# dscripka/openWakeWord

Measured on NVIDIA H100. Metric: 80ms audio-frames/sec (concurrent streams), higher is better.
Workload: dtype f16 operands / f32 accumulate (mel, BN, LayerNorm, sigmoid in f32; heads' first layer as fp16 hi/lo split = f32-grade)

## Files before the change

### include/owwb200.h

```cpp
#ifndef OWWB200_H
#define OWWB200_H

#include <stddef.h>
#include <stdint.h>

#ifdef __cplusplus
extern "C" {
#endif

#define OWW_OK            0
#define OWW_EINVAL      (-1)
#define OWW_ECUDA       (-2)
#define OWW_ENOMEM      (-3)
#define OWW_EUNSUPPORTED (-4)

#define OWW_SAMPLES_PER_CHUNK 1280
#define OWW_MEL_BINS            32
#define OWW_WINDOW_ROWS         76
#define OWW_EMBEDDING_DIM       96
#define OWW_INIT_FEATURE_ROWS   41
#define OWW_MAX_HEAD_LAYERS      8

#define OWW_CNN_FP32_WINDOW       0
#define OWW_CNN_TC_WINDOW         2
// ... 111 lines not shown
                      int32_t* h_staged, int16_t* d_staged, int64_t staged_stride, int16_t* d_hist, void* stream);
int oww_ingest_import(oww_ctx* ctx, const int32_t* h_stream_ids, int n, const int32_t* h_rates, const int64_t* h_consumed,
                      const int32_t* h_staged, const int16_t* d_staged, int64_t staged_stride, const int16_t* d_hist,
                      void* stream);

int oww_embed_clips(oww_ctx* ctx, const int16_t* d_pcm, int n_clips, int n_samples, float* d_emb, void* stream);
int oww_predict_clips(oww_ctx* ctx, const int16_t* d_pcm, int n_clips, int n_samples, int pad_samples,
                      const float* h_feature_init, int n_rows, float* d_scores, void* stream);
int oww_clip_schedule(int chunk_size, int64_t n_padded_samples, int32_t* h_chunks_per_call, int max);
int oww_predict_clips_ragged(oww_ctx* ctx, const int16_t* d_pcm, const int64_t* h_offsets, int n_clips, int pad_samples,
                             int chunk_size, const float* h_feature_init, int n_rows, float* d_scores, uint8_t* d_stepped,
                             float* d_emb, void* stream);
int oww_predict_clips_streams(oww_ctx* ctx, const int16_t* d_pcm, const int64_t* h_offsets, int n_clips, int pad_samples,
                              int chunk_size, const float* h_feature_init, int n_rows, float* d_scores, uint8_t* d_stepped,
                              float* d_emb, const int32_t* h_clip_streams, void* stream);
int oww_clip_slab_plan(oww_ctx* ctx, const int32_t* h_steps, int n_clips, int64_t* h_steps_computed, int64_t* h_steps_needed);
int oww_resample_clip_plan(int rate, int64_t n_in, int pad_samples, int64_t* n_out);
int oww_resample_clips(oww_ctx* ctx, const int16_t* d_in, const int64_t* h_in_offsets, const int32_t* h_rates, int n_clips,
                       int pad_samples, int16_t* d_out, const int64_t* h_out_offsets, void* stream);

typedef struct oww_mix_params {
    int32_t fg, bg, rir;
    int32_t reserved;
    int64_t fg_start, fg_len;
    int64_t bg_offset;
    int64_t start;
    double snr_db;
    double volume;
} oww_mix_params;
int oww_mix_clips(oww_ctx* ctx, const int16_t* d_fg, const int64_t* h_fg_off, int n_fg,
                  const int16_t* d_bg, const int64_t* h_bg_off, int n_bg,
                  const float* d_rir, const int64_t* h_rir_off, int n_rir,
                  const oww_mix_params* h_params, int n_mix, int64_t n_samples,
                  int16_t* d_out, uint8_t* d_valid, void* stream);

int oww_metrics_false_positives(oww_ctx* ctx, const float* d_scores, int64_t series_stride, int n_series, int n_frames,
                                const double* h_thresholds, int n_thresholds, int grouping_window, int32_t* h_counts, void* stream);
int oww_metrics_false_positives_f64(oww_ctx* ctx, const double* d_scores, int64_t series_stride, int n_series, int n_frames,
                                    const double* h_thresholds, int n_thresholds, int grouping_window, int32_t* h_counts,
                                    void* stream);
int oww_metrics_count_ge(oww_ctx* ctx, const float* d_scores, int64_t n, const double* h_thresholds, int n_thresholds,
                         uint64_t* h_counts, void* stream);
int oww_metrics_count_ge_f64(oww_ctx* ctx, const double* d_scores, int64_t n, const double* h_thresholds, int n_thresholds,
                             uint64_t* h_counts, void* stream);

int oww_debug_layer(oww_ctx* ctx, const float* d_windows, int n, int layer, float* d_out, void* stream);

int oww_debug_inc_plan(oww_ctx* ctx, int group, int n_streams, int32_t* out, int max_ints);
int oww_debug_inc_cut_plan(oww_ctx* ctx, int group, int n_streams, int n_layers, int32_t* out, int max_ints);

int oww_debug_inc_clocks(oww_ctx* ctx, int64_t* h_unused);
int oww_debug_inc_clocks_read(oww_ctx* ctx, int64_t* h_out104);
int oww_debug_heads_clocks(oww_ctx* ctx, int64_t* h_out64);

int oww_peer_alloc(oww_ctx* ctx, size_t bytes, void** d_ptr, unsigned char handle_out[64]);
int oww_peer_free(oww_ctx* ctx, void* d_ptr);
int oww_peer_open(oww_ctx* ctx, const unsigned char handle[64], void** d_ptr);
int oww_peer_close(oww_ctx* ctx, void* d_ptr);
int oww_peer_copy(oww_ctx* ctx, void* d_dst, const void* d_src, size_t bytes, void* stream);
int oww_peer_signal(oww_ctx* ctx, uint64_t* d_flag, uint64_t value, void* stream);
int oww_peer_wait(oww_ctx* ctx, const uint64_t* d_flags, int n, int stride, uint64_t value, double timeout_s, void* stream);
int oww_peer_status(oww_ctx* ctx, int* timed_out);

uint64_t oww_launch_count(const oww_ctx* ctx);
int oww_enable_stage_timing(oww_ctx* ctx, int n_slots);
int oww_stage_ms(oww_ctx* ctx, float out_ms[3]);

#ifdef __cplusplus
}
#endif
#endif
```

### openwakeword_b200/_native.py

```python
import ctypes as C
import os

import numpy as np

_HERE = os.path.dirname(os.path.abspath(__file__))
LIB_PATH = os.path.join(_HERE, "csrc", "libowwb200.so")
MAX_HEAD_LAYERS = 8

CNN_FP32_WINDOW = 0
CNN_FP32_INCREMENTAL = 1
CNN_TC_WINDOW = 2
CNN_TC_INCREMENTAL = 3


class Config(C.Structure):
    _fields_ = [("device", C.c_int32), ("max_chunks", C.c_int32), ("cnn_mode", C.c_int32),
                ("window_batch", C.c_int32), ("reserved", C.c_int32 * 4)]


class HeadDesc(C.Structure):
    _fields_ = [("n_in", C.c_int32), ("n_layers", C.c_int32), ("dims", C.c_int32 * (MAX_HEAD_LAYERS + 1)),
                ("layernorm", C.c_int32), ("final_act", C.c_int32)]


# ... 28 lines not shown
    "oww_fit_verifiers": (C.c_int, [_P, _P, C.c_int64, C.c_int, _P, _P, _P, C.c_int, C.c_double, C.c_int, C.c_double,
                                    _P, _P, _P, _P, _P, _P, _P]),
    "oww_load_verifiers": (C.c_int, [_P, C.c_int, _P, C.c_int, _P, _P, _P, _P]),
    "oww_add_head_bank": (C.c_int, [_P, C.POINTER(HeadDesc), C.c_int, C.POINTER(C.c_int)]),
    "oww_load_bank_head": (C.c_int, [_P, C.c_int, C.c_int, _P, C.c_size_t]),
    "oww_assign_bank_head": (C.c_int, [_P, C.c_int, _P, C.c_int, _P, _P]),
    "oww_set_head_bank_clip_slot": (C.c_int, [_P, C.c_int, C.c_int]),
    "oww_bank_head_predict": (C.c_int, [_P, C.c_int, C.c_int, _P, C.c_int, _P, _P]),
    "oww_n_heads": (C.c_int, [_P]),
    "oww_n_outputs": (C.c_int, [_P]),
    "oww_melspectrogram": (C.c_int, [_P, _P, C.c_int, C.c_int, _P, C.c_int, _P]),
    "oww_embed_windows": (C.c_int, [_P, _P, C.c_int, _P, _P]),
    "oww_head_predict": (C.c_int, [_P, C.c_int, _P, C.c_int, _P, _P]),
    "oww_set_streams": (C.c_int, [_P, C.c_int]),
    "oww_n_streams": (C.c_int, [_P]),
    "oww_reset": (C.c_int, [_P, _P, C.c_int, _P, C.c_int]),
    "oww_reset_async": (C.c_int, [_P, _P, C.c_int, _P, C.c_int, _P]),
    "oww_step": (C.c_int, [_P, _P, C.c_int64, C.c_int, _P, _P]),
    "oww_step_host": (C.c_int, [_P, _P, C.c_int64, C.c_int, _P]),
    "oww_step_host_submit": (C.c_int, [_P, _P, C.c_int64, C.c_int, C.POINTER(C.c_int)]),
    "oww_step_host_collect": (C.c_int, [_P, C.c_int, _P]),
    "oww_step_ragged": (C.c_int, [_P, _P, C.c_int64, _P, _P, _P]),
    "oww_step_host_ragged": (C.c_int, [_P, _P, C.c_int64, _P, _P]),
    "oww_step_host_ragged_submit": (C.c_int, [_P, _P, C.c_int64, _P, C.POINTER(C.c_int)]),
    "oww_get_features": (C.c_int, [_P, C.c_int, C.c_int, C.c_int, _P]),
    "oww_get_mel": (C.c_int, [_P, C.c_int, C.c_int, _P]),
    "oww_get_counts": (C.c_int, [_P, C.c_int, C.POINTER(C.c_int), C.POINTER(C.c_int)]),
    "oww_stream_state_info": (C.c_int, [_P, C.POINTER(C.c_size_t), C.POINTER(C.c_uint64)]),
    "oww_export_streams": (C.c_int, [_P, _P, C.c_int, _P, _P]),
    "oww_import_streams": (C.c_int, [_P, _P, C.c_int, _P, _P]),
    "oww_stream_state_status": (C.c_int, [_P, C.POINTER(C.c_int)]),
    "oww_set_detector": (C.c_int, [_P, C.POINTER(DetectLabel), C.c_int, C.c_double]),
    "oww_detect": (C.c_int, [_P, _P, C.c_int, _P, _P, _P, C.c_int, _P, _P]),
    "oww_detect_clips": (C.c_int, [_P, C.POINTER(DetectLabel), C.c_int, C.c_double, _P, _P, C.c_float, _P, C.c_int, C.c_int,
                                   _P, _P, C.c_int, _P, _P]),
    "oww_detector_export": (C.c_int, [_P, _P, C.c_int, _P, _P, _P]),
    "oww_detector_import": (C.c_int, [_P, _P, C.c_int, _P, _P, _P]),
    "oww_set_audio_history": (C.c_int, [_P, C.c_int]),
    "oww_get_audio": (C.c_int, [_P, _P, _P, C.c_int, C.c_int, _P, _P, _P]),
    "oww_capture_events": (C.c_int, [_P, _P, _P, C.c_int, C.c_int, _P, _P, _P]),
    "oww_audio_export": (C.c_int, [_P, _P, C.c_int, _P, _P, _P]),
    "oww_audio_import": (C.c_int, [_P, _P, C.c_int, _P, _P, _P]),
    "oww_set_input_rates": (C.c_int, [_P, _P, C.c_int, _P, _P]),
    "oww_ingest": (C.c_int, [_P, _P, _P, _P, _P, _P, _P]),
    "oww_ingest_capacity": (C.c_int, [_P, _P]),
    "oww_ingest_plan": (C.c_int, [C.c_int, C.c_int, C.c_int64, C.c_int, C.c_int64, C.POINTER(C.c_int64),
                                  C.POINTER(C.c_int32), C.POINTER(C.c_int32), C.POINTER(C.c_int64)]),
    "oww_resampler_taps": (C.c_int, [C.c_int, _P, C.c_int, C.POINTER(C.c_int), C.POINTER(C.c_int)]),
    "oww_ingest_export": (C.c_int, [_P, _P, C.c_int, _P, _P, _P, _P, C.c_int64, _P, _P]),
    "oww_ingest_import": (C.c_int, [_P, _P, C.c_int, _P, _P, _P, _P, C.c_int64, _P, _P]),
    "oww_embed_clips": (C.c_int, [_P, _P, C.c_int, C.c_int, _P, _P]),
    "oww_predict_clips": (C.c_int, [_P, _P, C.c_int, C.c_int, C.c_int, _P, C.c_int, _P, _P]),
    "oww_clip_schedule": (C.c_int, [C.c_int, C.c_int64, _P, C.c_int]),
    "oww_predict_clips_ragged": (C.c_int, [_P, _P, _P, C.c_int, C.c_int, C.c_int, _P, C.c_int, _P, _P, _P, _P]),
    "oww_predict_clips_streams": (C.c_int, [_P, _P, _P, C.c_int, C.c_int, C.c_int, _P, C.c_int, _P, _P, _P, _P, _P]),
    "oww_clip_slab_plan": (C.c_int, [_P, _P, C.c_int, C.POINTER(C.c_int64), C.POINTER(C.c_int64)]),
    "oww_resample_clip_plan": (C.c_int, [C.c_int, C.c_int64, C.c_int, C.POINTER(C.c_int64)]),
    "oww_resample_clips": (C.c_int, [_P, _P, _P, _P, C.c_int, C.c_int, _P, _P, _P]),
    "oww_mix_clips": (C.c_int, [_P, _P, _P, C.c_int, _P, _P, C.c_int, _P, _P, C.c_int, _P, C.c_int, C.c_int64, _P, _P, _P]),
    "oww_debug_layer": (C.c_int, [_P, _P, C.c_int, C.c_int, _P, _P]),
    "oww_debug_inc_plan": (C.c_int, [_P, C.c_int, C.c_int, _P, C.c_int]),
    "oww_debug_inc_cut_plan": (C.c_int, [_P, C.c_int, C.c_int, C.c_int, _P, C.c_int]),
    "oww_debug_inc_clocks": (C.c_int, [_P, _P]),
    "oww_debug_inc_clocks_read": (C.c_int, [_P, _P]),
    "oww_debug_heads_clocks": (C.c_int, [_P, _P]),
    "oww_peer_alloc": (C.c_int, [_P, C.c_size_t, C.POINTER(C.c_void_p), C.c_char_p]),
    "oww_peer_free": (C.c_int, [_P, _P]),
    "oww_peer_open": (C.c_int, [_P, C.c_char_p, C.POINTER(C.c_void_p)]),
    "oww_peer_close": (C.c_int, [_P, _P]),
    "oww_peer_copy": (C.c_int, [_P, _P, _P, C.c_size_t, _P]),
    "oww_peer_signal": (C.c_int, [_P, _P, C.c_uint64, _P]),
    "oww_peer_wait": (C.c_int, [_P, _P, C.c_int, C.c_int, C.c_uint64, C.c_double, _P]),
    "oww_peer_status": (C.c_int, [_P, C.POINTER(C.c_int)]),
    "oww_metrics_false_positives": (C.c_int, [_P, _P, C.c_int64, C.c_int, C.c_int, _P, C.c_int, C.c_int, _P, _P]),
    "oww_metrics_false_positives_f64": (C.c_int, [_P, _P, C.c_int64, C.c_int, C.c_int, _P, C.c_int, C.c_int, _P, _P]),
    "oww_metrics_count_ge": (C.c_int, [_P, _P, C.c_int64, _P, C.c_int, _P, _P]),
    "oww_metrics_count_ge_f64": (C.c_int, [_P, _P, C.c_int64, _P, C.c_int, _P, _P]),
    "oww_launch_count": (C.c_uint64, [_P]),
    "oww_enable_stage_timing": (C.c_int, [_P, C.c_int]),
    "oww_stage_ms": (C.c_int, [_P, _P]),
}
EXPORTED_SYMBOLS = tuple(_SIGNATURES)

_lib = None


def load_library():
    global _lib
    if _lib is not None:
        return _lib
    if not os.path.exists(LIB_PATH):
        raise ImportError(
            f"{LIB_PATH} is missing: the CUDA extension has not been built. Run "
            "`python -c 'import __graft_entry__ as g; g.build()'` at the repo root (nvcc, sm_90a). "
            "There is no CPU fallback for the b200 backend.")
    lib = C.CDLL(LIB_PATH)
    for name, (res, args) in _SIGNATURES.items():
        fn = getattr(lib, name)
        fn.restype = res
        fn.argtypes = args
    _lib = lib
    return lib


class NativeError(RuntimeError):
    pass


class ArgumentError(NativeError, ValueError):
    """A buffer the library would read or write out of bounds, refused in Python before the call.  A ValueError, and a
    NativeError like the library's own refusal of a short stride, so callers that catch either keep working."""


def clip_schedule(chunk_size, n_padded_samples):
    lib = load_library()
    n = lib.oww_clip_schedule(int(chunk_size), int(n_padded_samples), None, 0)
    if n < 0:
        raise NativeError(f"oww_clip_schedule failed ({n}): {lib.oww_last_error(None).decode()}")
    out = np.zeros(n, np.int32)
    if n:
        lib.oww_clip_schedule(int(chunk_size), int(n_padded_samples), _ptr(out), n)
    return out


def clip_slab_plan(steps, ctx=None):
    lib = load_library()
    st = np.ascontiguousarray(steps, np.int32)
    done, need = C.c_int64(0), C.c_int64(0)
    n = lib.oww_clip_slab_plan(ctx, _ptr(st), st.size, C.byref(done), C.byref(need))
    if n < 0:
        raise NativeError(f"oww_clip_slab_plan failed ({n})")
    return n, done.value, need.value


def resampler_taps(rate):
    lib = load_library()
    up, down = C.c_int(0), C.c_int(0)
    n = lib.oww_resampler_taps(int(rate), None, 0, C.byref(up), C.byref(down))
    if n < 0:
        raise ValueError(f"sample rate {rate} Hz is not supported: the input rates are 8000, 11025, 12000, 16000, 22050, "
                         "24000, 32000, 44100 and 48000 Hz")
    taps = np.zeros(n, np.float32)
    if n:
        lib.oww_resampler_taps(int(rate), _ptr(taps), n, None, None)
    return taps, up.value, down.value


def ingest_plan(rate, max_chunks, n_before, staged, n_in):
    lib = load_library()
    n_out, chunks, after, max_in = C.c_int64(0), C.c_int32(0), C.c_int32(0), C.c_int64(0)
    rc = lib.oww_ingest_plan(int(rate), int(max_chunks), int(n_before), int(staged), int(n_in), C.byref(n_out),
                             C.byref(chunks), C.byref(after), C.byref(max_in))
    if rc and n_in <= max_in.value:
        raise ValueError(f"oww_ingest_plan refused rate {rate}")
    if rc:
        return None, None, None, max_in.value
    return n_out.value, chunks.value, after.value, max_in.value


def resample_clip_plan(rate, n_in, pad_samples):
    lib = load_library()
    n = C.c_int64(0)
    if lib.oww_resample_clip_plan(int(rate), int(n_in), int(pad_samples), C.byref(n)):
        raise ValueError(f"oww_resample_clip_plan refused rate {rate}, {n_in} samples, pad {pad_samples}: the rates are "
                         "8000, 11025, 12000, 16000, 22050, 24000, 32000, 44100 and 48000 Hz, and the padding a multiple "
                         "of 640 samples (40 ms)")
    return n.value


def _ptr(a):
    if a is None:
        return None
    if isinstance(a, int):
        return a
    if isinstance(a, np.ndarray):
        return a.ctypes.data
    return a.data_ptr()
# ... 700 lines not shown
```

### openwakeword_b200/csrc/heads_grp.cu

```cuda
#include "oww_internal.h"
#include "heads_mma.cuh"
#include <algorithm>
#include <cmath>
#include <cstring>

namespace {

constexpr int kHgThreads = 9 * 32;
constexpr int kHgTile = 128;
constexpr int kHgMaxStages = 6;
constexpr int kHgChunkK = 32;
constexpr int kHgAPlane = 4 * kHgTile * 16;
constexpr int kHgABytes = 2 * kHgAPlane;
constexpr int kHgTileBytes = 3 * kHgABytes;
constexpr int kHgSmem = 227 * 1024;
constexpr int kHgRing0 = 1024;

__device__ __forceinline__ void hg_warp_wait(uint32_t bar, uint32_t parity, int lane) {
    if (lane == 0) mbar_wait(bar, parity);
    __syncwarp();
}
__device__ __forceinline__ void hg_split8(const float* x, uint4& hi, uint4& lo) { hm_split8(x, hi, lo); }

__global__ void __launch_bounds__(256) feat16_sync_kernel(const float* __restrict__ ring, int64_t ring_stride, int rows_mask,
                                                          const int* __restrict__ count, const int* __restrict__ ids, int n,
                                                          int depth, int pos, int NS, int n_tiles, uint8_t* __restrict__ out) {
    const int64_t total = (int64_t)n * 12 * depth;
    oww_pdl_sync();
    for (int64_t i = (int64_t)blockIdx.x * 256 + threadIdx.x; i < total; i += (int64_t)gridDim.x * 256) {
        const int lb = (int)(i % n);
        const int j = (int)((i / n) % 12);
        const int k = (int)(i / ((int64_t)n * 12));
        const int b = ids ? ids[lb] : lb;
        const int row = count[b] - 1 - k;
        float x[8];
        if (row >= 0) {
            const float4* p = reinterpret_cast<const float4*>(ring + (int64_t)b * ring_stride + (int64_t)(row & rows_mask) * 96 + j * 8);
            const float4 u = __ldcg(p), v = __ldcg(p + 1);
            x[0] = u.x; x[1] = u.y; x[2] = u.z; x[3] = u.w; x[4] = v.x; x[5] = v.y; x[6] = v.z; x[7] = v.w;
        } else {
#pragma unroll
            for (int e = 0; e < 8; ++e) x[e] = 0.f;
        }
        uint4 hi, lo;
        hg_split8(x, hi, lo);
        int slot = (pos - k) % NS;
        if (slot < 0) slot += NS;
        const int tile = b >> 7, r = b & 127, q = j >> 2, o = j & 3;
        uint8_t* t = out + ((int64_t)slot * n_tiles + tile) * kHgTileBytes + q * kHgABytes + (o * kHgTile + r) * 16;
        *reinterpret_cast<uint4*>(t) = hi;
        *reinterpret_cast<uint4*>(t + kHgAPlane) = lo;
    }
}

__global__ void __launch_bounds__(256) feat16_linear_kernel(const float* __restrict__ feats, int64_t clip_stride, int n_clips,
                                                            int n_rows, int pad, int n_tiles, uint8_t* __restrict__ out) {
    const int64_t total = (int64_t)n_clips * 12 * n_rows;
    for (int64_t i = (int64_t)blockIdx.x * 256 + threadIdx.x; i < total; i += (int64_t)gridDim.x * 256) {
        const int b = (int)(i % n_clips);
        const int j = (int)((i / n_clips) % 12);
        const int t = (int)(i / ((int64_t)n_clips * 12));
        const float4* p = reinterpret_cast<const float4*>(feats + (int64_t)b * clip_stride + (int64_t)t * 96 + j * 8);
        const float4 u = __ldcg(p), v = __ldcg(p + 1);
        const float x[8] = {u.x, u.y, u.z, u.w, v.x, v.y, v.z, v.w};
        uint4 hi, lo;
        hg_split8(x, hi, lo);
        const int tile = b >> 7, r = b & 127, q = j >> 2, o = j & 3;
        uint8_t* d = out + ((int64_t)(pad + t) * n_tiles + tile) * kHgTileBytes + q * kHgABytes + (o * kHgTile + r) * 16;
        *reinterpret_cast<uint4*>(d) = hi;
        *reinterpret_cast<uint4*>(d + kHgAPlane) = lo;
    }
}

using HgLayer = HmLayer;
struct HgHead {
    HeadDev dev;
    const uint8_t* w;
    HgLayer L[OWW_MAX_HEAD_LAYERS];
};
struct HgGroup {
    int head, n_in, n_tot;
    const uint8_t* w0;
    uint32_t w0_bytes;
    int stages; uint32_t stage_bytes;
    int cpr;
};
struct HeadsGrpArgs {
    HgHead head[16];
    HgGroup grp[8];
    const uint8_t* f16; int n_tiles, NS, slot_end;
    int steps;
    int n; float* out; int out_stride, combine_max, n_terms;
    long long* dbg;
};

__global__ void __launch_bounds__(kHgThreads, 1) heads_grp_kernel(const __grid_constant__ HeadsGrpArgs a) {
    extern __shared__ __align__(128) uint8_t smem[];
    const HgGroup& G = a.grp[blockIdx.y];
    const int tile = blockIdx.x, s0 = tile * kHgTile;
    const int S = G.stages;
    uint64_t* bars = reinterpret_cast<uint64_t*>(smem);
    uint8_t* ring = smem + kHgRing0;
    const int warp = __shfl_sync(0xffffffffu, (int)(threadIdx.x >> 5), 0);
    const int lane = threadIdx.x & 31;
    const uint32_t bar0 = smem_u32(bars);
    auto full = [&](int s) { return bar0 + 8u * s; };
    auto empty = [&](int s) { return bar0 + 8u * (kHgMaxStages + s); };
    const uint32_t acc_done = bar0 + 8u * (2 * kHgMaxStages);
    const uint32_t wn_full = acc_done + 8u;
    if (threadIdx.x == 0) {
        for (int s = 0; s < kHgMaxStages; ++s) { mbar_init(full(s), 1); mbar_init(empty(s), 8); }
        mbar_init(acc_done, 8);
        mbar_init(wn_full, 1);
        asm volatile("fence.mbarrier_init.release.cluster;" ::: "memory");
    }
    __syncthreads();
    const bool split = a.n_terms >= 3;
    const int cpr = G.cpr;
    const int n_in = G.n_in, n_tot = G.n_tot, n_terms = a.n_terms;
    const int n_it = n_in * 3 / cpr;
    const HgHead& HH = a.head[G.head];
    const uint32_t stage_bytes = G.stage_bytes, w0_bytes = G.w0_bytes;
    const uint32_t ring_u = smem_u32(ring);
    const uint32_t w_next = ring_u + 2 * kHmBufBytes;
    long long* dbg = (a.dbg && blockIdx.x == 0) ? a.dbg + 8 * blockIdx.y : nullptr;
    if (dbg && threadIdx.x == 0) dbg[0] = clock64();
    pdl_trigger();
    pdl_wait();

    if (warp == 8) {
        if (lane == 0) {
            const int NS = a.NS, n_tiles = a.n_tiles;
            int slot = (a.slot_end + (a.steps > 0 ? (int)blockIdx.z : 0) - n_in + 1) % NS;
            if (slot < 0) slot += NS;
            const uint8_t* f16 = a.f16 + (int64_t)tile * kHgTileBytes;
            const uint8_t* w0 = G.w0;
            const int64_t slot_pitch = (int64_t)n_tiles * kHgTileBytes;
            uint32_t stage = 0, par = 1, st = ring_u;
            const uint32_t a_off = (uint32_t)cpr * kHgABytes;
            const uint32_t a_bytes = split ? kHgABytes : kHgAPlane, w_bytes = split ? w0_bytes : w0_bytes / 2;
            for (int c = 0; c < n_in; ++c) {
                const uint8_t* arow = f16 + (int64_t)slot * slot_pitch;
                for (int q = 0; q < 3; q += cpr) {
                    mbar_wait(empty(stage), par);
                    mbar_expect_tx(full(stage), (uint32_t)cpr * (a_bytes + w_bytes));
                    for (int k = 0; k < cpr; ++k) {
                        bulk_g2s(st + k * kHgABytes, arow + (q + k) * kHgABytes, a_bytes, full(stage));
                        bulk_g2s(st + a_off + k * w0_bytes, w0 + (size_t)k * w0_bytes, w_bytes, full(stage));
                    }
                    w0 += (size_t)cpr * w0_bytes;
                    st += stage_bytes;
                    if (++stage == (uint32_t)S) { stage = 0; par ^= 1u; st = ring_u; }
                }
                if (++slot == NS) slot = 0;
            }
            if (dbg) dbg[1] = clock64();
            for (int l = 1; l < HH.dev.n_layers; ++l) {
                mbar_wait(acc_done, (uint32_t)((l - 1) & 1));
                const uint32_t wb = split ? HH.L[l].w_bytes : HH.L[l].w_bytes / 2;
                mbar_expect_tx(wn_full, wb);
                bulk_g2s(w_next, HH.w + HH.L[l].w_off, wb, wn_full);
            }
        }
    } else {
        const int wg = warp >> 2;
        float acc[64];
        const uint32_t w_plane = (uint32_t)n_tot * 64u;
        wg_dispatch_n(n_tot, [&](auto nc) { dispatch_int<3, 1>(cpr, [&](auto cc) { dispatch_int<3, 1>(n_terms, [&](auto tc) {
            constexpr int NN = decltype(nc)::value, CPR = decltype(cc)::value, PER_CHUNK = 2 * decltype(tc)::value;
            float d[NN / 2];
            uint32_t stage = 0, par = 0, st = ring_u;
            for (int it = 0; it < n_it; ++it) {
                hg_warp_wait(full(stage), par, lane);
                wg_fence();
#pragma unroll
                for (int s = 0; s < CPR * PER_CHUNK; ++s) {
                    const int k = s / PER_CHUNK, r = s - k * PER_CHUNK, t = r >> 1, ks = r & 1;
                    const uint32_t ab = st + (uint32_t)k * kHgABytes + (uint32_t)wg * kHmAPlane, wb = st + (uint32_t)cpr * kHgABytes + (uint32_t)k * w0_bytes;
                    const uint32_t au = ab + (t == 1 ? (uint32_t)kHgAPlane : 0u);
                    const uint32_t wu = wb + (t == 2 ? w_plane : 0u);
                    const uint64_t ad = make_desc(au + (uint32_t)(2 * ks) * (kHgTile * 16), kHgTile * 16, 128u);
                    const uint64_t bd = make_desc(wu + (uint32_t)(2 * ks) * (uint32_t)NN * 16u, (uint32_t)NN * 16u, 128u);
                    wg_mma<NN>(d, ad, bd, (it | s) != 0);
                }
                wg_commit();
                wg_wait_all();
                __syncwarp();
                if (lane == 0) mbar_arrive(empty(stage));
                st += stage_bytes;
                if (++stage == (uint32_t)S) { stage = 0; par ^= 1u; st = ring_u; }
            }
#pragma unroll
            for (int k = 0; k < NN / 2; ++k) acc[k] = d[k];
        }); }); });
        __syncwarp();
        if (lane == 0) mbar_arrive(acc_done);
        if (dbg && threadIdx.x == 0) dbg[2] = clock64();
        const int r = threadIdx.x & 127, sr = s0 + wg * kHmRows + r;
        float* o = nullptr;
        if (r < kHmRows && sr < a.n) {
            const int64_t orow = a.steps > 0 ? (int64_t)sr * a.steps + blockIdx.z : (int64_t)sr;
            o = a.out + orow * a.out_stride + HH.dev.col0;
        }
        named_bar_sync(3, 256);
        hm_layers(acc, n_tot, HH.dev, HH.L, n_terms, ring + wg * kHmBufBytes, w_next, wn_full, acc_done, 1 + wg, o,
                  a.combine_max);
        if (dbg && threadIdx.x == 0) dbg[4] = clock64();
    }
}

}

struct oww_heads_grp {
    HeadsGrpArgs args;
    int n_groups = 0;
    uint32_t covered = 0;
    std::vector<void*> d_w0;
    long long* d_dbg = nullptr;
    uint8_t* d_f16_bulk = nullptr; size_t bulk_bytes = 0;
    uint8_t* d_f16 = nullptr;
    int NS = 0, n_tiles = 0, depth = 0;
    long pos = 0;
    bool mirror_valid = false;
    size_t n_heads_built = 0;
};

void oww_heads_grp_free(oww_ctx* ctx) {
    oww_heads_grp* g = ctx->heads_grp;
    if (!g) return;
    for (void* p : g->d_w0) cudaFree(p);
    cudaFree(g->d_f16); cudaFree(g->d_dbg); cudaFree(g->d_f16_bulk);
    delete g;
    ctx->heads_grp = nullptr;
}

void oww_heads_grp_drop_mirror(oww_ctx* ctx) {
    oww_heads_grp* g = ctx->heads_grp;
    if (!g) return;
    cudaFree(g->d_f16); g->d_f16 = nullptr; g->mirror_valid = false;
}

void oww_feat16_invalidate(oww_ctx* ctx) {
    if (ctx->heads_grp) ctx->heads_grp->mirror_valid = false;
}

static int hg_build(oww_ctx* ctx) {
    oww_heads_grp_free(ctx);
    oww_heads_grp* g = new oww_heads_grp();
    ctx->heads_grp = g;
    g->n_heads_built = ctx->heads.size();
    HeadsGrpArgs& a = g->args;
    std::memset(&a, 0, sizeof(a));
    const int nh = (int)ctx->heads.size();
    if (nh > 16) return OWW_OK;
    std::vector<int> cand;
    for (int i = 0; i < nh; ++i)
        if (oww_heads_tc_supported(ctx, i) && !ctx->heads[i].tc_w0_host.empty()) cand.push_back(i);
    auto colw = [&](int i) { int w = 16; for (const auto& T : ctx->heads[i].tc_layers) w = std::max(w, T.NP); return w; };
    std::sort(cand.begin(), cand.end(), [&](int x, int y) {
        const int nx = ctx->heads[x].desc.n_in, ny = ctx->heads[y].desc.n_in;
        if (nx != ny) return nx > ny;
        const int cx = colw(x), cy = colw(y);
        return cx != cy ? cx > cy : x < y;
    });
    for (int i : cand) {
        if (g->n_groups >= 8) break;
        HgGroup& G = a.grp[g->n_groups];
        std::memset(&G, 0, sizeof(G));
        const Head& h = ctx->heads[i];
        G.head = i;
        G.n_in = h.desc.n_in;
        HgHead& HH = a.head[i];
        HeadDev& d = HH.dev;
        d.blob = h.d_blob;
        d.n_in = h.desc.n_in; d.n_layers = h.desc.n_layers; d.layernorm = h.desc.layernorm; d.final_act = h.desc.final_act;
        uint32_t wn_max = 0;
        for (int l = 0; l <= h.desc.n_layers; ++l) d.dims[l] = h.desc.dims[l];
        for (int l = 0; l < h.desc.n_layers; ++l) {
            d.w_off[l] = (int)h.w_off[l]; d.b_off[l] = (int)h.b_off[l];
            d.g_off[l] = (int)h.g_off[l]; d.h_off[l] = (int)h.h_off[l];
            const Head::TcLayer& T = h.tc_layers[l];
            HH.L[l] = HgLayer{T.K, T.D, T.Kp, T.NP, T.w_off, T.w_bytes, T.unscale};
            if (l >= 1) wn_max = std::max(wn_max, T.w_bytes);
        }
        d.col0 = h.col0;
        HH.w = reinterpret_cast<const uint8_t*>(h.d_w1_tc);
        G.n_tot = colw(i);
        G.w0_bytes = (uint32_t)(2 * 4 * G.n_tot * 16);
        G.cpr = 2 * 3 * (kHgABytes + (int)G.w0_bytes) <= kHgSmem - kHgRing0 ? 3 : 1;
        G.stage_bytes = (uint32_t)(G.cpr * (kHgABytes + (int)G.w0_bytes));
        G.stages = std::min(kHgMaxStages, (kHgSmem - kHgRing0) / (int)G.stage_bytes);
        const bool fits = G.stages >= 2 && 2 * (size_t)kHmBufBytes + ((wn_max + 127u) & ~127u) <= (size_t)(kHgSmem - kHgRing0);
        if (!fits) continue;
        const size_t blk = (size_t)G.w0_bytes / 2;
        std::vector<__half> packed((size_t)G.n_in * 3 * blk, __float2half(0.f));
        const int D = h.desc.dims[1];
        const float sc = 1.0f / h.tc_layers[0].unscale;
        const float* w = h.tc_w0_host.data();
        for (int c = 0; c < G.n_in; ++c)
            for (int q = 0; q < 3; ++q) {
                __half* dst = packed.data() + ((size_t)c * 3 + q) * blk;
                for (int o = 0; o < 4; ++o)
                    for (int n = 0; n < D; ++n)
                        for (int e = 0; e < 8; ++e) {
                            const int kk = c * 96 + q * kHgChunkK + o * 8 + e;
                            const float v = w[(size_t)kk * D + n] * sc;
                            const __half hi = __float2half_rn(v);
                            const size_t at = ((size_t)o * G.n_tot + n) * 8 + e;
                            dst[at] = hi;
                            dst[at + blk / 2] = __float2half_rn(v - __half2float(hi));
                        }
            }
        void* dw = nullptr;
        OWW_CUDA(ctx, cudaMalloc(&dw, packed.size() * sizeof(__half)));
        g->d_w0.push_back(dw);
        OWW_CUDA(ctx, cudaMemcpy(dw, packed.data(), packed.size() * sizeof(__half), cudaMemcpyHostToDevice));
        G.w0 = reinterpret_cast<const uint8_t*>(dw);
        g->covered |= 1u << i;
        g->depth = std::max(g->depth, G.n_in);
        ++g->n_groups;
    }
    std::sort(a.grp, a.grp + g->n_groups, [](const HgGroup& x, const HgGroup& y) {
        return (int64_t)x.n_in * x.n_tot > (int64_t)y.n_in * y.n_tot;
    });
    if (g->n_groups) OWW_CUDA(ctx, cudaFuncSetAttribute(heads_grp_kernel, cudaFuncAttributeMaxDynamicSharedMemorySize, kHgSmem));
    return OWW_OK;
}

static int hg_ensure(oww_ctx* ctx) {
    if (!ctx->heads_grp || ctx->heads_grp->n_heads_built != ctx->heads.size()) return hg_build(ctx);
    return OWW_OK;
}

static int hg_sync(oww_ctx* ctx, const int* d_ids, int n, int depth, cudaStream_t s) {
    oww_heads_grp* g = ctx->heads_grp;
    const int64_t total = (int64_t)n * 12 * depth;
    if (total <= 0) return OWW_OK;
    const unsigned grid = (unsigned)std::min<int64_t>((total + 255) / 256, (int64_t)ctx->sm_count * 16);
    OWW_CUDA(ctx, oww_launch_pdl(ctx->late_pdl, feat16_sync_kernel, dim3(grid), dim3(256), 0, s, (const float*)ctx->d_feat_ring,
                                 (int64_t)ctx->feat_rows * 96, ctx->feat_rows - 1, (const int*)ctx->d_feat_count, d_ids, n, depth,
                                 (int)(g->pos % g->NS), g->NS, g->n_tiles, g->d_f16));
    OWW_LAUNCH_CHECK(ctx);
    return OWW_OK;
}

int oww_feat16_advance(oww_ctx* ctx, int n_chunks, cudaStream_t s) {
    if (!ctx->tc_heads || ctx->cfg.cnn_mode == OWW_CNN_FP32_WINDOW || ctx->heads.empty() || !ctx->grp_heads) return OWW_OK;
    int rc = hg_ensure(ctx);
    if (rc) return rc;
    oww_heads_grp* g = ctx->heads_grp;
    if (!g->n_groups) return OWW_OK;
    const int need_ns = g->depth + ctx->cfg.max_chunks;
    if (!g->d_f16 || g->NS < need_ns) {
        cudaFree(g->d_f16); g->d_f16 = nullptr;
        g->NS = need_ns;
        g->n_tiles = (ctx->n_streams + kHgTile - 1) / kHgTile;
        const size_t bytes = (size_t)g->NS * g->n_tiles * kHgTileBytes;
        OWW_CUDA(ctx, cudaMalloc(&g->d_f16, bytes));
        OWW_CUDA(ctx, cudaMemsetAsync(g->d_f16, 0, bytes, s));
        g->mirror_valid = false;
    }
    if (!g->mirror_valid) {
        g->pos = g->NS;
        g->mirror_valid = true;
        return hg_sync(ctx, nullptr, ctx->n_streams, g->depth + ctx->cfg.max_chunks - 1, s);
    }
    g->pos += n_chunks;
    if (g->pos > (1L << 40)) g->pos = g->pos % g->NS + g->NS;
    return hg_sync(ctx, nullptr, ctx->n_streams, n_chunks, s);
}

int oww_feat16_resync(oww_ctx* ctx, const int* d_ids, int n, cudaStream_t s) {
    oww_heads_grp* g = ctx->heads_grp;
    if (!g || !g->d_f16 || !g->mirror_valid) return OWW_OK;
    return hg_sync(ctx, d_ids, n, g->depth + ctx->cfg.max_chunks - 1, s);
}

uint32_t oww_heads_grp_covered(oww_ctx* ctx) {
    oww_heads_grp* g = ctx->heads_grp;
    if (!g || !g->mirror_valid || !g->n_groups || g->n_heads_built != ctx->heads.size()) return 0;
    return g->covered;
}

int oww_heads_grp_launch(oww_ctx* ctx, int back, int n, float* d_out, int out_stride, int combine_max, cudaStream_t s) {
    oww_heads_grp* g = ctx->heads_grp;
    HeadsGrpArgs& a = g->args;
    a.f16 = g->d_f16; a.n_tiles = g->n_tiles; a.NS = g->NS;
    a.slot_end = (int)((g->pos - back) % g->NS);
    a.n = n; a.out = d_out; a.out_stride = out_stride; a.combine_max = combine_max;
    a.n_terms = ctx->tc_heads_terms;
    a.dbg = g->d_dbg;
    a.steps = 0;
    dim3 grid((n + kHgTile - 1) / kHgTile, g->n_groups);
    OWW_CUDA(ctx, oww_launch_pdl(ctx->late_pdl, heads_grp_kernel, grid, dim3(kHgThreads), kHgSmem, s, a));
    OWW_LAUNCH_CHECK(ctx);
    return OWW_OK;
}

uint32_t oww_heads_grp_bulk(oww_ctx* ctx, const FeatSrc& src, int n, float* d_out, int out_stride, cudaStream_t s, int* rc_out) {
    *rc_out = OWW_OK;
    if (!ctx->tc_heads || !ctx->grp_heads || ctx->cfg.cnn_mode == OWW_CNN_FP32_WINDOW || src.count || src.steps <= 0) return 0;
    if ((*rc_out = hg_ensure(ctx))) return 0;
    oww_heads_grp* g = ctx->heads_grp;
    if (!g->n_groups || src.steps > 65535 || n % src.steps) return 0;
    const int m = n / src.steps, n_rows = (int)(src.stride / 96), pad = g->depth;
    if (src.row0 + src.steps > n_rows) return 0;
    const int n_tiles = (m + kHgTile - 1) / kHgTile;
    const size_t bytes = (size_t)(pad + n_rows) * n_tiles * kHgTileBytes;
    auto fail = [&](cudaError_t e) { *rc_out = oww_fail(ctx, OWW_ECUDA, "bulk feature mirror: %s", cudaGetErrorString(e)); return 0u; };
    cudaError_t e;
    if (g->bulk_bytes < bytes) {
        cudaFree(g->d_f16_bulk); g->d_f16_bulk = nullptr; g->bulk_bytes = 0;
        if ((e = cudaMalloc(&g->d_f16_bulk, bytes)) != cudaSuccess) return fail(e);
        g->bulk_bytes = bytes;
    }
    if ((e = cudaMemsetAsync(g->d_f16_bulk, 0, bytes, s)) != cudaSuccess) return fail(e);
    {
        const int64_t total = (int64_t)m * 12 * n_rows;
        const unsigned grid = (unsigned)std::min<int64_t>((total + 255) / 256, (int64_t)ctx->sm_count * 32);
        feat16_linear_kernel<<<grid, 256, 0, s>>>(src.base, src.stride, m, n_rows, pad, n_tiles, g->d_f16_bulk);
        ctx->launches++;
    }
    HeadsGrpArgs& a = g->args;
    a.f16 = g->d_f16_bulk; a.n_tiles = n_tiles; a.NS = pad + n_rows;
    a.slot_end = pad + src.row0;
    a.steps = src.steps;
    a.n = m; a.out = d_out; a.out_stride = out_stride; a.combine_max = 0;
    a.n_terms = ctx->tc_heads_terms;
    a.dbg = nullptr;
    dim3 grid(n_tiles, g->n_groups, src.steps);
    heads_grp_kernel<<<grid, kHgThreads, kHgSmem, s>>>(a);
    ctx->launches++;
    if ((e = cudaGetLastError()) != cudaSuccess) return fail(e);
    return g->covered;
}

extern "C" int oww_debug_heads_clocks(oww_ctx* ctx, int64_t* h_out64) {
    oww_heads_grp* g = ctx ? ctx->heads_grp : nullptr;
    if (!g) return OWW_EINVAL;
    if (!g->d_dbg) {
        OWW_CUDA(ctx, cudaMalloc(&g->d_dbg, 256 * sizeof(long long)));
        OWW_CUDA(ctx, cudaMemset(g->d_dbg, 0, 256 * sizeof(long long)));
        return OWW_OK;
    }
    OWW_CUDA(ctx, cudaDeviceSynchronize());
    OWW_CUDA(ctx, cudaMemcpy(h_out64, g->d_dbg, 256 * sizeof(long long), cudaMemcpyDeviceToHost));
    return OWW_OK;
}
```

### openwakeword_b200/csrc/heads_mma.cuh

```cuda
#pragma once
#include "tc_common.cuh"

namespace {

constexpr int kHmRows = 64;
constexpr int kHmAPlane = kHmRows * 16;
constexpr int kHmPitch = 129;
constexpr int kHmRowScale = 128;
constexpr int kHmHBytes = (kHmRows * kHmPitch * 4 + 127) & ~127;
constexpr int kHmABytes = 2 * 16 * kHmAPlane;
constexpr int kHmPBytes = 3 * 128 * 4;
constexpr int kHmBufBytes = kHmHBytes + kHmABytes + kHmPBytes;

struct HmLayer { int K, D, Kp, NP; uint32_t w_off, w_bytes; float unscale; };

__device__ __forceinline__ void hm_split8(const float* x, uint4& hi, uint4& lo) {
    __half2 h[4], l[4];
#pragma unroll
    for (int e = 0; e < 4; ++e) {
        const __half h0 = __float2half_rn(x[2 * e]), h1 = __float2half_rn(x[2 * e + 1]);
        h[e] = __halves2half2(h0, h1);
        l[e] = __floats2half2_rn(x[2 * e] - __half2float(h0), x[2 * e + 1] - __half2float(h1));
    }
    hi = *reinterpret_cast<uint4*>(h);
    lo = *reinterpret_cast<uint4*>(l);
}

__device__ __forceinline__ void hm_layers(float* acc, int n0, const HeadDev& H, const HmLayer* L, int n_terms, uint8_t* buf,
                                          uint32_t w_next, uint32_t wn_full, uint32_t acc_done, int bar, float* o, int combine_max) {
    const int tid = threadIdx.x & 127, wq = tid >> 5, lane = tid & 31, q = lane & 3;
    float* hbuf = reinterpret_cast<float*>(buf);
    uint8_t* a_next = buf + kHmHBytes;
    float* prm = reinterpret_cast<float*>(buf + kHmHBytes + kHmABytes);
    const int n_layers = H.n_layers;
    int ncols = n0;
    for (int l = 0; l < n_layers; ++l) {
        const int D = L[l].D;
        const float us = L[l].unscale;
        if (tid < D) {
            prm[tid] = __ldg(H.blob + H.b_off[l] + tid);
            if (H.layernorm && l < n_layers - 1) {
                prm[128 + tid] = __ldg(H.blob + H.g_off[l] + tid);
                prm[256 + tid] = __ldg(H.blob + H.h_off[l] + tid);
            }
        }
        named_bar_sync(bar, 128);
        const int row0 = 16 * wq + (lane >> 2);
        const float us0 = l ? us * hbuf[row0 * kHmPitch + kHmRowScale] : us;
        const float us1 = l ? us * hbuf[(row0 + 8) * kHmPitch + kHmRowScale] : us;
#pragma unroll
        for (int k = 0; k < 64; ++k) {
            const int j = k >> 2, i = (k >> 1) & 1, e = k & 1;
            const int col = 8 * j + 2 * q + e, row = row0 + 8 * i;
            if (8 * j < ncols && col < D) hbuf[row * kHmPitch + col] = fmaf(acc[k], i ? us1 : us0, prm[col]);
        }
        named_bar_sync(bar, 128);
        float* hrow = hbuf + tid * kHmPitch;
        if (l == n_layers - 1) {
            if (tid < kHmRows && o) {
                const int n_out = D;
                if (H.final_act == 4) {
                    for (int d = 0; d < n_out; ++d) hrow[d] = fmaxf(hrow[d], 0.f);
                } else if (H.final_act == 1) {
                    for (int d = 0; d < n_out; ++d) hrow[d] = 1.0f / (1.0f + expf(-hrow[d]));
                } else if (H.final_act == 2 || H.final_act == 3) {
                    float m = -INFINITY;
                    for (int d = 0; d < n_out; ++d) {
                        if (H.final_act == 3) hrow[d] = fmaxf(hrow[d], 0.f);
                        m = fmaxf(m, hrow[d]);
                    }
                    float sum = 0.f;
                    for (int d = 0; d < n_out; ++d) { hrow[d] = expf(hrow[d] - m); sum += hrow[d]; }
                    for (int d = 0; d < n_out; ++d) hrow[d] = hrow[d] / sum;
                }
                for (int d = 0; d < n_out; ++d) o[d] = combine_max ? fmaxf(o[d], hrow[d]) : hrow[d];
            }
            break;
        }
        const HmLayer& N = L[l + 1];
        if (tid < kHmRows) {
            float mu = 0.f, rstd = 1.f;
            if (H.layernorm) {
                float sum = 0.f;
                for (int d = 0; d < D; ++d) sum += hrow[d];
                mu = sum / (float)D;
                float sq = 0.f;
                for (int d = 0; d < D; ++d) { const float c = hrow[d] - mu; sq = fmaf(c, c, sq); }
                rstd = 1.0f / sqrtf(sq / (float)D + 1e-5f);
            }
            const float* g = prm + 128;
            const float* hb = prm + 256;
            float vmax = 0.f;
            for (int d = 0; d < D; ++d) {
                float v = hrow[d];
                if (H.layernorm) v = (v - mu) * rstd * g[d] + hb[d];
                v = fmaxf(v, 0.f);
                hrow[d] = v;
                vmax = fmaxf(vmax, v);
            }
            const int ex = oww_scale_exponent_of_max(vmax, -100, 100);
            const float up = ldexpf(1.f, ex);
            hrow[kHmRowScale] = ldexpf(1.f, -ex);
            for (int j = 0; j < N.Kp / 8; ++j) {
                float x[8];
#pragma unroll
                for (int e = 0; e < 8; ++e) {
                    const int d = j * 8 + e;
                    x[e] = d < D ? hrow[d] * up : 0.f;
                }
                uint4 hi, lo;
                hm_split8(x, hi, lo);
                *reinterpret_cast<uint4*>(a_next + j * kHmAPlane + tid * 16) = hi;
                if (n_terms >= 2) *reinterpret_cast<uint4*>(a_next + 16 * kHmAPlane + j * kHmAPlane + tid * 16) = lo;
            }
        }
        asm volatile("fence.proxy.async.shared::cta;" ::: "memory");
        named_bar_sync(bar, 128);
        mbar_wait(wn_full, (uint32_t)(l & 1));
        const uint32_t a_lo = smem_u32(a_next);
        const uint32_t a_unit[2] = {a_lo, a_lo + 16u * kHmAPlane};
        const uint32_t w_unit[2] = {w_next, w_next + N.w_bytes / 2};
        wg_dispatch_n(N.NP, [&](auto nc) {
            dispatch_int<8, 4, 2, 6, 1, 3, 5, 7>(N.Kp / 16, [&](auto kc) {
                dispatch_int<3, 1>(n_terms, [&](auto tc) {
                    constexpr int NN = decltype(nc)::value, NK = decltype(kc)::value, NT = decltype(tc)::value;
                    float d[NN / 2];
                    wg_fence();
#pragma unroll
                    for (int s = 0; s < NT * NK; ++s) {
                        const int t = s / NK, kq = s - t * NK;
                        const uint32_t au = a_unit[t == 1 ? 1 : 0], wu = w_unit[t == 2 ? 1 : 0];
                        const uint64_t ad = make_desc(au + (uint32_t)(2 * kq) * kHmAPlane, kHmAPlane, 128u);
                        const uint64_t bd = make_desc(wu + (uint32_t)(2 * kq * NN) * 16u, (uint32_t)NN * 16u, 128u);
                        wg_mma<NN>(d, ad, bd, s > 0);
                    }
                    wg_commit();
                    wg_wait_all();
#pragma unroll
                    for (int k = 0; k < NN / 2; ++k) acc[k] = d[k];
                });
            });
        });
        __syncwarp();
        if (lane == 0) mbar_arrive(acc_done);
        ncols = N.NP;
    }
}

}
```

Measured before the change: 6.200 million.

## Pair 64-wide heads sharing input depth into one grouped first-layer GEMM

Heads whose first layer is 64 columns wide and that share the same input depth are merged into a single group. Their first-layer weights are packed side by side into a 128-column MMA, so the feature tiles are streamed once for both heads. Afterwards the tail layers of each head run in turn, with half the accumulator stashed in shared memory in between. The grid is flattened to 1D with a custom item ordering that walks extra groups in reverse tile order. This adds shared-memory stash pressure and mbarrier parity bookkeeping across the two heads.

```diff
diff --git a/include/owwb200.h b/include/owwb200.h
--- a/include/owwb200.h
+++ b/include/owwb200.h
@@ -187,6 +187,7 @@
 int oww_debug_inc_clocks(oww_ctx* ctx, int64_t* h_unused);
 int oww_debug_inc_clocks_read(oww_ctx* ctx, int64_t* h_out104);
 int oww_debug_heads_clocks(oww_ctx* ctx, int64_t* h_out64);
+int64_t oww_heads_grp_items(int n_tiles, int steps, int n_groups, int32_t* h_out, int64_t max_items);
 
 int oww_peer_alloc(oww_ctx* ctx, size_t bytes, void** d_ptr, unsigned char handle_out[64]);
 int oww_peer_free(oww_ctx* ctx, void* d_ptr);
diff --git a/openwakeword_b200/_native.py b/openwakeword_b200/_native.py
--- a/openwakeword_b200/_native.py
+++ b/openwakeword_b200/_native.py
@@ -104,6 +104,7 @@
     "oww_embed_clips": (C.c_int, [_P, _P, C.c_int, C.c_int, _P, _P]),
     "oww_predict_clips": (C.c_int, [_P, _P, C.c_int, C.c_int, C.c_int, _P, C.c_int, _P, _P]),
     "oww_clip_schedule": (C.c_int, [C.c_int, C.c_int64, _P, C.c_int]),
+    "oww_heads_grp_items": (C.c_int64, [C.c_int, C.c_int, C.c_int, _P, C.c_int64]),
     "oww_predict_clips_ragged": (C.c_int, [_P, _P, _P, C.c_int, C.c_int, C.c_int, _P, C.c_int, _P, _P, _P, _P]),
     "oww_predict_clips_streams": (C.c_int, [_P, _P, _P, C.c_int, C.c_int, C.c_int, _P, C.c_int, _P, _P, _P, _P, _P]),
     "oww_clip_slab_plan": (C.c_int, [_P, _P, C.c_int, C.POINTER(C.c_int64), C.POINTER(C.c_int64)]),
@@ -175,6 +176,17 @@
     return out
 
 
+def heads_grp_items(n_tiles, steps, n_groups):
+    lib = load_library()
+    n = lib.oww_heads_grp_items(int(n_tiles), int(steps), int(n_groups), None, 0)
+    if n < 0:
+        raise NativeError(f"oww_heads_grp_items failed ({n})")
+    out = np.zeros((n, 3), np.int32)
+    if n:
+        lib.oww_heads_grp_items(int(n_tiles), int(steps), int(n_groups), _ptr(out), n)
+    return out
+
+
 def clip_slab_plan(steps, ctx=None):
     lib = load_library()
     st = np.ascontiguousarray(steps, np.int32)
diff --git a/openwakeword_b200/csrc/heads_grp.cu b/openwakeword_b200/csrc/heads_grp.cu
--- a/openwakeword_b200/csrc/heads_grp.cu
+++ b/openwakeword_b200/csrc/heads_grp.cu
@@ -15,6 +15,7 @@
 constexpr int kHgTileBytes = 3 * kHgABytes;
 constexpr int kHgSmem = 227 * 1024;
 constexpr int kHgRing0 = 1024;
+constexpr int kHgStash = 256 * 32 * 4;
 
 __device__ __forceinline__ void hg_warp_wait(uint32_t bar, uint32_t parity, int lane) {
     if (lane == 0) mbar_wait(bar, parity);
@@ -79,7 +80,7 @@
     HgLayer L[OWW_MAX_HEAD_LAYERS];
 };
 struct HgGroup {
-    int head, n_in, n_tot;
+    int head, head2, n_in, n_tot;
     const uint8_t* w0;
     uint32_t w0_bytes;
     int stages; uint32_t stage_bytes;
@@ -88,16 +89,30 @@
 struct HeadsGrpArgs {
     HgHead head[16];
     HgGroup grp[8];
+    int n_groups;
     const uint8_t* f16; int n_tiles, NS, slot_end;
     int steps;
     int n; float* out; int out_stride, combine_max, n_terms;
     long long* dbg;
 };
 
+struct HgItem { int tile, step, group; };
+__host__ __device__ __forceinline__ HgItem hg_item(int i, int n_units, int steps, int n_groups) {
+    int u = i, g = 0;
+    if (i >= n_units) {
+        const int j = i - n_units, m = n_groups - 1;
+        u = n_units - 1 - j / m;
+        g = 1 + j % m;
+    }
+    return {u / steps, u % steps, g};
+}
+
 __global__ void __launch_bounds__(kHgThreads, 1) heads_grp_kernel(const __grid_constant__ HeadsGrpArgs a) {
     extern __shared__ __align__(128) uint8_t smem[];
-    const HgGroup& G = a.grp[blockIdx.y];
-    const int tile = blockIdx.x, s0 = tile * kHgTile;
+    const int steps = a.steps > 0 ? a.steps : 1;
+    const HgItem I = hg_item((int)blockIdx.x, (a.n + kHgTile - 1) / kHgTile * steps, steps, a.n_groups);
+    const HgGroup& G = a.grp[I.group];
+    const int tile = I.tile, s0 = tile * kHgTile;
     const int S = G.stages;
     uint64_t* bars = reinterpret_cast<uint64_t*>(smem);
     uint8_t* ring = smem + kHgRing0;
@@ -123,7 +138,7 @@
     const uint32_t stage_bytes = G.stage_bytes, w0_bytes = G.w0_bytes;
     const uint32_t ring_u = smem_u32(ring);
     const uint32_t w_next = ring_u + 2 * kHmBufBytes;
-    long long* dbg = (a.dbg && blockIdx.x == 0) ? a.dbg + 8 * blockIdx.y : nullptr;
+    long long* dbg = (a.dbg && tile == 0 && I.step == 0) ? a.dbg + 8 * I.group : nullptr;
     if (dbg && threadIdx.x == 0) dbg[0] = clock64();
     pdl_trigger();
     pdl_wait();
@@ -131,7 +146,7 @@
     if (warp == 8) {
         if (lane == 0) {
             const int NS = a.NS, n_tiles = a.n_tiles;
-            int slot = (a.slot_end + (a.steps > 0 ? (int)blockIdx.z : 0) - n_in + 1) % NS;
+            int slot = (a.slot_end + I.step - n_in + 1) % NS;
             if (slot < 0) slot += NS;
             const uint8_t* f16 = a.f16 + (int64_t)tile * kHgTileBytes;
             const uint8_t* w0 = G.w0;
@@ -155,11 +170,15 @@
                 if (++slot == NS) slot = 0;
             }
             if (dbg) dbg[1] = clock64();
-            for (int l = 1; l < HH.dev.n_layers; ++l) {
-                mbar_wait(acc_done, (uint32_t)((l - 1) & 1));
-                const uint32_t wb = split ? HH.L[l].w_bytes : HH.L[l].w_bytes / 2;
-                mbar_expect_tx(wn_full, wb);
-                bulk_g2s(w_next, HH.w + HH.L[l].w_off, wb, wn_full);
+            uint32_t ph = 0;
+            for (int h = 0; h < (G.head2 >= 0 ? 2 : 1); ++h) {
+                const HgHead& HL = a.head[h ? G.head2 : G.head];
+                for (int l = 1; l < HL.dev.n_layers; ++l, ++ph) {
+                    mbar_wait(acc_done, ph & 1u);
+                    const uint32_t wb = split ? HL.L[l].w_bytes : HL.L[l].w_bytes / 2;
+                    mbar_expect_tx(wn_full, wb);
+                    bulk_g2s(w_next, HL.w + HL.L[l].w_off, wb, wn_full);
+                }
             }
         }
     } else {
@@ -199,12 +218,33 @@
         const int r = threadIdx.x & 127, sr = s0 + wg * kHmRows + r;
         float* o = nullptr;
         if (r < kHmRows && sr < a.n) {
-            const int64_t orow = a.steps > 0 ? (int64_t)sr * a.steps + blockIdx.z : (int64_t)sr;
-            o = a.out + orow * a.out_stride + HH.dev.col0;
+            const int64_t orow = a.steps > 0 ? (int64_t)sr * a.steps + I.step : (int64_t)sr;
+            o = a.out + orow * a.out_stride;
         }
         named_bar_sync(3, 256);
-        hm_layers(acc, n_tot, HH.dev, HH.L, n_terms, ring + wg * kHmBufBytes, w_next, wn_full, acc_done, 1 + wg, o,
-                  a.combine_max);
+        uint8_t* buf = ring + wg * kHmBufBytes;
+        if (G.head2 < 0) {
+            hm_layers(acc, n_tot, HH.dev, HH.L, n_terms, buf, w_next, wn_full, acc_done, 1 + wg, o ? o + HH.dev.col0 : nullptr,
+                      a.combine_max);
+        } else {
+            float4* stash = reinterpret_cast<float4*>(smem + kHgSmem - kHgStash) + threadIdx.x;
+#pragma unroll
+            for (int k = 0; k < 8; ++k) {
+                stash[256 * k] = make_float4(acc[32 + 4 * k], acc[33 + 4 * k], acc[34 + 4 * k], acc[35 + 4 * k]);
+                acc[32 + 4 * k] = acc[33 + 4 * k] = acc[34 + 4 * k] = acc[35 + 4 * k] = 0.f;
+            }
+            const HgHead& H2 = a.head[G.head2];
+            hm_layers(acc, 64, HH.dev, HH.L, n_terms, buf, w_next, wn_full, acc_done, 1 + wg, o ? o + HH.dev.col0 : nullptr,
+                      a.combine_max);
+#pragma unroll
+            for (int k = 0; k < 8; ++k) {
+                const float4 v = stash[256 * k];
+                acc[4 * k] = v.x; acc[1 + 4 * k] = v.y; acc[2 + 4 * k] = v.z; acc[3 + 4 * k] = v.w;
+                acc[32 + 4 * k] = acc[33 + 4 * k] = acc[34 + 4 * k] = acc[35 + 4 * k] = 0.f;
+            }
+            hm_layers(acc, 64, H2.dev, H2.L, n_terms, buf, w_next, wn_full, acc_done, 1 + wg, o ? o + H2.dev.col0 : nullptr,
+                      a.combine_max, (uint32_t)(HH.dev.n_layers - 1) & 1u);
+        }
         if (dbg && threadIdx.x == 0) dbg[4] = clock64();
     }
 }
@@ -263,13 +303,9 @@
         const int cx = colw(x), cy = colw(y);
         return cx != cy ? cx > cy : x < y;
     });
+    std::vector<uint32_t> wn_grp(8, 0);
     for (int i : cand) {
-        if (g->n_groups >= 8) break;
-        HgGroup& G = a.grp[g->n_groups];
-        std::memset(&G, 0, sizeof(G));
         const Head& h = ctx->heads[i];
-        G.head = i;
-        G.n_in = h.desc.n_in;
         HgHead& HH = a.head[i];
         HeadDev& d = HH.dev;
         d.blob = h.d_blob;
@@ -285,44 +321,74 @@
         }
         d.col0 = h.col0;
         HH.w = reinterpret_cast<const uint8_t*>(h.d_w1_tc);
-        G.n_tot = colw(i);
-        G.w0_bytes = (uint32_t)(2 * 4 * G.n_tot * 16);
-        G.cpr = 2 * 3 * (kHgABytes + (int)G.w0_bytes) <= kHgSmem - kHgRing0 ? 3 : 1;
-        G.stage_bytes = (uint32_t)(G.cpr * (kHgABytes + (int)G.w0_bytes));
-        G.stages = std::min(kHgMaxStages, (kHgSmem - kHgRing0) / (int)G.stage_bytes);
-        const bool fits = G.stages >= 2 && 2 * (size_t)kHmBufBytes + ((wn_max + 127u) & ~127u) <= (size_t)(kHgSmem - kHgRing0);
+        HgGroup* P = g->n_groups ? &a.grp[g->n_groups - 1] : nullptr;
+        const bool pair = P && P->head2 < 0 && P->n_tot == 64 && colw(i) == 64 && P->n_in == h.desc.n_in;
+        if (!pair && g->n_groups >= 8) continue;
+        HgGroup T;
+        if (pair) {
+            T = *P;
+            T.head2 = i;
+            T.n_tot = 128;
+            wn_max = std::max(wn_max, wn_grp[g->n_groups - 1]);
+        } else {
+            std::memset(&T, 0, sizeof(T));
+            T.head = i; T.head2 = -1;
+            T.n_in = h.desc.n_in;
+            T.n_tot = colw(i);
+        }
+        T.w0_bytes = (uint32_t)(2 * 4 * T.n_tot * 16);
+        T.cpr = 2 * 3 * (kHgABytes + (int)T.w0_bytes) <= kHgSmem - kHgRing0 ? 3 : 1;
+        T.stage_bytes = (uint32_t)(T.cpr * (kHgABytes + (int)T.w0_bytes));
+        T.stages = std::min(kHgMaxStages, (kHgSmem - kHgRing0) / (int)T.stage_bytes);
+        const size_t later = 2 * (size_t)kHmBufBytes + ((wn_max + 127u) & ~127u) + (pair ? kHgStash : 0);
+        const bool fits = T.stages >= 2 && later <= (size_t)(kHgSmem - kHgRing0) &&
+                          (!pair || (size_t)T.stages * T.stage_bytes <= (size_t)(kHgSmem - kHgRing0 - kHgStash));
         if (!fits) continue;
+        if (pair) {
+            *P = T;
+            wn_grp[g->n_groups - 1] = wn_max;
+        } else {
+            a.grp[g->n_groups] = T;
+            wn_grp[g->n_groups] = wn_max;
+            ++g->n_groups;
+        }
+        g->covered |= 1u << i;
+        g->depth = std::max(g->depth, T.n_in);
+    }
+    for (int k = 0; k < g->n_groups; ++k) {
+        HgGroup& G = a.grp[k];
         const size_t blk = (size_t)G.w0_bytes / 2;
         std::vector<__half> packed((size_t)G.n_in * 3 * blk, __float2half(0.f));
-        const int D = h.desc.dims[1];
-        const float sc = 1.0f / h.tc_layers[0].unscale;
-        const float* w = h.tc_w0_host.data();
-        for (int c = 0; c < G.n_in; ++c)
-            for (int q = 0; q < 3; ++q) {
-                __half* dst = packed.data() + ((size_t)c * 3 + q) * blk;
-                for (int o = 0; o < 4; ++o)
-                    for (int n = 0; n < D; ++n)
-                        for (int e = 0; e < 8; ++e) {
-                            const int kk = c * 96 + q * kHgChunkK + o * 8 + e;
-                            const float v = w[(size_t)kk * D + n] * sc;
-                            const __half hi = __float2half_rn(v);
-                            const size_t at = ((size_t)o * G.n_tot + n) * 8 + e;
-                            dst[at] = hi;
-                            dst[at + blk / 2] = __float2half_rn(v - __half2float(hi));
-                        }
-            }
+        for (int m = 0; m < (G.head2 >= 0 ? 2 : 1); ++m) {
+            const Head& h = ctx->heads[m ? G.head2 : G.head];
+            const int D = h.desc.dims[1], n0 = 64 * m;
+            const float sc = 1.0f / h.tc_layers[0].unscale;
+            const float* w = h.tc_w0_host.data();
+            for (int c = 0; c < G.n_in; ++c)
+                for (int q = 0; q < 3; ++q) {
+                    __half* dst = packed.data() + ((size_t)c * 3 + q) * blk;
+                    for (int o = 0; o < 4; ++o)
+                        for (int n = 0; n < D; ++n)
+                            for (int e = 0; e < 8; ++e) {
+                                const int kk = c * 96 + q * kHgChunkK + o * 8 + e;
+                                const float v = w[(size_t)kk * D + n] * sc;
+                                const __half hi = __float2half_rn(v);
+                                const size_t at = ((size_t)o * G.n_tot + n0 + n) * 8 + e;
+                                dst[at] = hi;
+                                dst[at + blk / 2] = __float2half_rn(v - __half2float(hi));
+                            }
+                }
+        }
         void* dw = nullptr;
         OWW_CUDA(ctx, cudaMalloc(&dw, packed.size() * sizeof(__half)));
         g->d_w0.push_back(dw);
         OWW_CUDA(ctx, cudaMemcpy(dw, packed.data(), packed.size() * sizeof(__half), cudaMemcpyHostToDevice));
         G.w0 = reinterpret_cast<const uint8_t*>(dw);
-        g->covered |= 1u << i;
-        g->depth = std::max(g->depth, G.n_in);
-        ++g->n_groups;
     }
     std::sort(a.grp, a.grp + g->n_groups, [](const HgGroup& x, const HgGroup& y) {
         return (int64_t)x.n_in * x.n_tot > (int64_t)y.n_in * y.n_tot;
     });
+    a.n_groups = g->n_groups;
     if (g->n_groups) OWW_CUDA(ctx, cudaFuncSetAttribute(heads_grp_kernel, cudaFuncAttributeMaxDynamicSharedMemorySize, kHgSmem));
     return OWW_OK;
 }
@@ -382,6 +448,16 @@
     return g->covered;
 }
 
+extern "C" int64_t oww_heads_grp_items(int n_tiles, int steps, int n_groups, int32_t* out, int64_t max_items) {
+    if (n_tiles < 0 || steps < 1 || n_groups < 1 || (int64_t)n_tiles * steps * n_groups > INT32_MAX) return OWW_EINVAL;
+    const int64_t items = (int64_t)n_tiles * steps * n_groups;
+    for (int64_t i = 0; out && i < std::min(items, max_items); ++i) {
+        const HgItem I = hg_item((int)i, n_tiles * steps, steps, n_groups);
+        out[3 * i] = I.tile; out[3 * i + 1] = I.step; out[3 * i + 2] = I.group;
+    }
+    return items;
+}
+
 int oww_heads_grp_launch(oww_ctx* ctx, int back, int n, float* d_out, int out_stride, int combine_max, cudaStream_t s) {
     oww_heads_grp* g = ctx->heads_grp;
     HeadsGrpArgs& a = g->args;
@@ -391,7 +467,7 @@
     a.n_terms = ctx->tc_heads_terms;
     a.dbg = g->d_dbg;
     a.steps = 0;
-    dim3 grid((n + kHgTile - 1) / kHgTile, g->n_groups);
+    const dim3 grid((unsigned)(((n + kHgTile - 1) / kHgTile) * g->n_groups));
     OWW_CUDA(ctx, oww_launch_pdl(ctx->late_pdl, heads_grp_kernel, grid, dim3(kHgThreads), kHgSmem, s, a));
     OWW_LAUNCH_CHECK(ctx);
     return OWW_OK;
@@ -428,8 +504,7 @@
     a.n = m; a.out = d_out; a.out_stride = out_stride; a.combine_max = 0;
     a.n_terms = ctx->tc_heads_terms;
     a.dbg = nullptr;
-    dim3 grid(n_tiles, g->n_groups, src.steps);
-    heads_grp_kernel<<<grid, kHgThreads, kHgSmem, s>>>(a);
+    heads_grp_kernel<<<(unsigned)(n_tiles * src.steps * g->n_groups), kHgThreads, kHgSmem, s>>>(a);
     ctx->launches++;
     if ((e = cudaGetLastError()) != cudaSuccess) return fail(e);
     return g->covered;
diff --git a/openwakeword_b200/csrc/heads_mma.cuh b/openwakeword_b200/csrc/heads_mma.cuh
--- a/openwakeword_b200/csrc/heads_mma.cuh
+++ b/openwakeword_b200/csrc/heads_mma.cuh
@@ -27,7 +27,8 @@
 }
 
 __device__ __forceinline__ void hm_layers(float* acc, int n0, const HeadDev& H, const HmLayer* L, int n_terms, uint8_t* buf,
-                                          uint32_t w_next, uint32_t wn_full, uint32_t acc_done, int bar, float* o, int combine_max) {
+                                          uint32_t w_next, uint32_t wn_full, uint32_t acc_done, int bar, float* o, int combine_max,
+                                          uint32_t wn_par = 0) {
     const int tid = threadIdx.x & 127, wq = tid >> 5, lane = tid & 31, q = lane & 3;
     float* hbuf = reinterpret_cast<float*>(buf);
     uint8_t* a_next = buf + kHmHBytes;
@@ -116,7 +117,7 @@
         }
         asm volatile("fence.proxy.async.shared::cta;" ::: "memory");
         named_bar_sync(bar, 128);
-        mbar_wait(wn_full, (uint32_t)(l & 1));
+        mbar_wait(wn_full, ((uint32_t)l ^ wn_par) & 1u);
         const uint32_t a_lo = smem_u32(a_next);
         const uint32_t a_unit[2] = {a_lo, a_lo + 16u * kHmAPlane};
         const uint32_t w_unit[2] = {w_next, w_next + N.w_bytes / 2};
```

Result: faster. 6.302 million, median of 6 (+1.6%).
